# farhad-dalirani/StereoVision-SLAM

Hardware: AMD Instinct MI355X
Metric: stereo frames/sec (track + local BA), KITTI-00-shaped synthetic stereo 1241x376 (620x188 after the reference's 1/2 decimation) (higher is better)
Workload: dtype u8/i32 fixed-point (pyramid, LK), f32 (GFTT), f64 (LM, BA)

## Files before the change

### stereovision-slam_amd/csrc/k_lk.h

```cpp
#pragma once
#include "dev_common.h"

struct LkJob { int prev_slot, next_slot, pt_ofs, npts; };
struct LkParams {
    int max_level;
    int max_count;
    double eps2;
    double min_eig_thr;
    int use_initial_flow;
    float eig_num_thr;
    int eig_use_div;
    int njobs, blocks_per_job;
};

#define LK_WIN 11
#define LK_NPIX 121
#define LK_W_BITS 14
#define LK_REG 32
#ifndef LK_WAVES_PER_BLOCK
#define LK_WAVES_PER_BLOCK 1
#endif
#define LK_IROW 20

typedef uint32_t lk_u32_ua __attribute__((aligned(1)));
typedef uint16_t lk_u16_ua __attribute__((aligned(1)));
typedef short lk_s2 __attribute__((ext_vector_type(2)));

__device__ __forceinline__ int lk_dot2(uint32_t a, uint32_t b, int c)
{
    int r;
    asm("v_dot2_i32_i16 %0, %1, %2, %3" : "=v"(r) : "v"(a), "v"(b), "v"(c));
    return r;
}
#define LK_PAIR_SEL0 0x0c010c00u
__device__ __forceinline__ uint32_t lk_pair_sel(int a) { return LK_PAIR_SEL0 + (uint32_t)(a & 3) * 0x00010001u; }
__device__ __forceinline__ uint32_t lk_pair_at(const uint32_t *base32, int a, uint32_t sel)
{
    const uint32_t *q = base32 + (a >> 2);
    return __builtin_amdgcn_perm(q[1], q[0], sel);
}

__device__ __forceinline__ int lk_floor_i(float x)
{
    int r;
    asm("v_cvt_flr_i32_f32 %0, %1" : "=v"(r) : "v"(x));
    return r;
}

struct LkW { uint32_t top, bot; };

__device__ __forceinline__ LkW lk_weights(float a, float b)
{
    typedef float lk_f2 __attribute__((ext_vector_type(2)));
    const float S = (float)(1 << LK_W_BITS), M = 12582912.f;
    const float A = a * S, An = S - A, bn = 1.f - b;
    const lk_f2 p0 = (lk_f2){An, A} * (lk_f2){bn, bn} + (lk_f2){M, M};
    const uint32_t b00 = __float_as_uint(p0.x), b01 = __float_as_uint(p0.y), b10 = __float_as_uint(An * b + M);
    const uint32_t w11 = ((1u << LK_W_BITS) + 3u * 0x4B400000u) - (b00 + b01 + b10);
    LkW w;
    w.top = __builtin_amdgcn_perm(b01, b00, 0x05040100u);
    w.bot = __builtin_amdgcn_perm(w11, b10, 0x05040100u);
    return w;
}

__device__ __forceinline__ int lk_sample_u8(const uint32_t *base32, int a, int row_stride, LkW w)
{
    const uint32_t sel = lk_pair_sel(a);
    const uint32_t *q = base32 + (a >> 2);
    const int rs = row_stride >> 2;
    const uint32_t t = __builtin_amdgcn_perm(q[1], q[0], sel), b = __builtin_amdgcn_perm(q[rs + 1], q[rs], sel);
    return lk_dot2(t, w.top, lk_dot2(b, w.bot, 1 << (LK_W_BITS - 5 - 1))) >> (LK_W_BITS - 5);
}

__device__ __forceinline__ int lk_sample_diff(const uint32_t *base32, int a, int row_stride, LkW w, int acc0)
{
    const uint32_t sel = lk_pair_sel(a);
    const uint32_t *q = base32 + (a >> 2);
    const int rs = row_stride >> 2;
    const uint32_t t = __builtin_amdgcn_perm(q[1], q[0], sel), b = __builtin_amdgcn_perm(q[rs + 1], q[rs], sel);
    return lk_dot2(t, w.top, lk_dot2(b, w.bot, acc0)) >> (LK_W_BITS - 5);
}

typedef const __attribute__((address_space(3))) uint32_t *lk_lds_u32;
__device__ __forceinline__ int lk_sample_diff_at(uint32_t addr, LkW w, int acc0)
{
    lk_lds_u32 q = (lk_lds_u32)(uintptr_t)addr;
    const uint32_t t = q[0], b = q[LK_REG];
    return lk_dot2(t, w.top, lk_dot2(b, w.bot, acc0)) >> (LK_W_BITS - 5);
}

struct LkJRegs { uint32_t v[4]; };
__device__ __forceinline__ LkJRegs lk_stage_J_issue(const uint8_t *J0, uint32_t lofs, int pitch, int w, int h,
                                                    int cx, int cy, int lane, int &rx0, int &ry0)
{
    rx0 = __builtin_amdgcn_readfirstlane((cx - 10) & ~3);
    ry0 = __builtin_amdgcn_readfirstlane(cy - 10);
    const int r = lane >> 3, c4 = lane & 7;
    LkJRegs o;
    if (rx0 >= -SVS_BORDER && rx0 + LK_REG <= w + SVS_BORDER && ry0 >= -SVS_BORDER && ry0 + LK_REG <= h + SVS_BORDER) {
        const uint32_t p = lofs + (uint32_t)((ry0 + r) * pitch + (rx0 + c4 * 4));
#pragma unroll
        for (int k = 0; k < 4; ++k)
            o.v[k] = *reinterpret_cast<const uint32_t *>(J0 + (p + (uint32_t)(8 * k * pitch)));
    } else {
        const int gxmax = (w + SVS_BORDER - 4) & ~3;
        const int gx = max(-SVS_BORDER, min(rx0 + c4 * 4, gxmax));
#pragma unroll
        for (int k = 0; k < 4; ++k) {
            const int gy = max(-SVS_BORDER, min(ry0 + r + 8 * k, h + SVS_BORDER - 1));
            o.v[k] = *reinterpret_cast<const uint32_t *>(J0 + (lofs + (uint32_t)(gy * pitch + gx)));
        }
    }
    return o;
}
__device__ __forceinline__ void lk_stage_J_commit(uint32_t *sJ, const LkJRegs &o, int lane)
{
    typedef uint32_t lk_u4 __attribute__((ext_vector_type(4)));
    const int r = lane >> 3, c4 = lane & 7;
#pragma unroll
    for (int k = 0; k < 4; ++k) {
        const uint32_t cur = o.v[k];
        const uint32_t nxt = (uint32_t)__builtin_amdgcn_update_dpp(0, (int)cur, 0x101 , 0xf, 0xf, true);
        lk_u4 pr;
        pr.x = __builtin_amdgcn_perm(nxt, cur, 0x0c010c00u);
        pr.y = __builtin_amdgcn_perm(nxt, cur, 0x0c020c01u);
        pr.z = __builtin_amdgcn_perm(nxt, cur, 0x0c030c02u);
        pr.w = __builtin_amdgcn_perm(nxt, cur, 0x0c040c03u);
        *reinterpret_cast<lk_u4 *>(sJ + (r + 8 * k) * LK_REG + 4 * c4) = pr;
    }
    __builtin_amdgcn_fence(__ATOMIC_RELEASE, "wavefront");
    __builtin_amdgcn_wave_barrier();
}
__device__ __forceinline__ void lk_stage_J(uint32_t *sJ, const uint8_t *J0, uint32_t lofs, int pitch, int w, int h,
                                           int cx, int cy, int lane, int &rx0, int &ry0)
{
    const LkJRegs o = lk_stage_J_issue(J0, lofs, pitch, w, h, cx, cy, lane, rx0, ry0);
    lk_stage_J_commit(sJ, o, lane);
}

__device__ __forceinline__ float lk_sum_to_f32(long long s, float scale)
{
    const int lo = (int)s;
    const bool fits = (long long)lo == s;
    const int t = fits ? lo : (int)((s >> 1) | (s & 1));
    const uint32_t kb = fits ? __float_as_uint(scale) : __float_as_uint(2.f * scale);
    return (float)t * __uint_as_float(kb);
}

typedef unsigned lk_u2 __attribute__((ext_vector_type(2)));
__device__ __forceinline__ int lk_row_reduce(int w)
{
    w += dpp_i32<SVS_DPP_XOR1>(w);
    w += dpp_i32<SVS_DPP_XOR2>(w);
    w += dpp_i32<SVS_DPP_HALF_MIRROR>(w);
    w += dpp_i32<SVS_DPP_MIRROR>(w);
    return w;
}
__device__ __forceinline__ void lk_wave_sum2_i32(int a, int b, int &sa, int &sb)
{
    const lk_u2 r = __builtin_amdgcn_permlane16_swap((unsigned)a, (unsigned)b, false, false);
    const int v = (int)(r.x + r.y);
    const int w = lk_row_reduce(v);
    sa = __builtin_amdgcn_readlane(w, 0) + __builtin_amdgcn_readlane(w, 32);
    sb = __builtin_amdgcn_readlane(w, 16) + __builtin_amdgcn_readlane(w, 48);
}
__device__ __forceinline__ void lk_wave_sum4_i32(int a, int b, int c, int d, int &sa, int &sb, int &sc, int &sd)
{
    const lk_u2 r1 = __builtin_amdgcn_permlane16_swap((unsigned)a, (unsigned)b, false, false);
    const lk_u2 r2 = __builtin_amdgcn_permlane16_swap((unsigned)c, (unsigned)d, false, false);
    const int v1 = (int)(r1.x + r1.y), v2 = (int)(r2.x + r2.y);
    const lk_u2 q = __builtin_amdgcn_permlane32_swap((unsigned)v1, (unsigned)v2, false, false);
    const int w = lk_row_reduce((int)(q.x + q.y));
    sa = __builtin_amdgcn_readlane(w, 0);
    sb = __builtin_amdgcn_readlane(w, 16);
    sc = __builtin_amdgcn_readlane(w, 32);
    sd = __builtin_amdgcn_readlane(w, 48);
}

#ifndef LK_OCC_TEST
#define LK_OCC_TEST 0
#endif
#if LK_OCC_TEST == 1
#define LK_OCC_ATTR __attribute__((amdgpu_waves_per_eu(8, 8)))
#else
#define LK_OCC_ATTR
#endif
__global__ void __launch_bounds__(64 * LK_WAVES_PER_BLOCK) LK_OCC_ATTR
k_lk(const LkJob *jobs, const uint8_t *pyr, PyrGeom g, const float2 *prev_xy, float2 *next_xy,
     uint8_t *status, float *err, LkParams prm)
{
    __shared__ uint32_t sI_all[LK_WAVES_PER_BLOCK][16 * LK_IROW / 4 + 2];
    __shared__ uint32_t sD_all[LK_WAVES_PER_BLOCK][144];
    __shared__ __attribute__((aligned(16))) uint32_t sJ_all[LK_WAVES_PER_BLOCK][LK_REG * LK_REG];

#if LK_OCC_TEST == 2
    __shared__ uint32_t sPad[8192];
    sPad[threadIdx.x] = threadIdx.x;
    if (prm.max_count < 0) status[0] = (uint8_t)sPad[(threadIdx.x * 37) & 8191];
#endif
    const int wave = threadIdx.x >> 6, lane = threadIdx.x & 63;
    const int slot = blockIdx.x >> 3, round = slot / prm.blocks_per_job;
    const int job = round * 8 + (blockIdx.x & 7);
    if (job >= prm.njobs) return;
    const LkJob jb = jobs[job];
    const int pi = (slot - round * prm.blocks_per_job) * LK_WAVES_PER_BLOCK + wave;
    if (pi >= jb.npts) return;
    const int pt = jb.pt_ofs + pi;
    uint32_t *sI32 = sI_all[wave];
    uint32_t *sD = sD_all[wave];
    uint32_t *sJ = sJ_all[wave];

    const uint8_t *slotI = pyr + (size_t)jb.prev_slot * g.slot_bytes;
    const uint8_t *slotJ = pyr + (size_t)jb.next_slot * g.slot_bytes;

    const float2 prevp = prev_xy[pt];
    float2 nextp = next_xy[pt];
    bool st = true;
    float errv = 0.f;

    const int p0 = lane, p1 = lane + 64;
    const bool has1 = p1 < LK_NPIX;
    const int wy0 = p0 / LK_WIN, wx0 = p0 - wy0 * LK_WIN;
    const int wy1 = has1 ? p1 / LK_WIN : 0, wx1 = has1 ? p1 - wy1 * LK_WIN : 0;
    const int oI0 = (wy0 + 1) * LK_IROW + wx0 + 1, oI1 = (wy1 + 1) * LK_IROW + wx1 + 1;
    const int oD0 = wy0 * 12 + wx0, oD1 = wy1 * 12 + wx1;
    const int oJ0 = wy0 * LK_REG + wx0, oJ1 = wy1 * LK_REG + wx1;
    const uint32_t aJ0 = (uint32_t)(uintptr_t)(__attribute__((address_space(3))) uint32_t *)sJ + 4u * (uint32_t)oJ0,
                   aJ1 = (uint32_t)(uintptr_t)(__attribute__((address_space(3))) uint32_t *)sJ + 4u * (uint32_t)oJ1;
    const int sr = lane >> 2, sc = (lane & 3) * 3;
    const float FLT_SCALE = 1.f / (float)(1 << 20);
    const float e_lo = (float)(prm.eps2 * (1.0 - 2e-6)), e_hi = (float)(prm.eps2 * (1.0 + 2e-6));

    int max_level = prm.max_level;
    if (max_level > g.nlevels - 1) max_level = g.nlevels - 1;

    for (int level = max_level; level >= 0; --level) {
        const int w = g.w[level], h = g.h[level], pitch = g.pitch[level];
        const uint32_t lofs = (uint32_t)g.ofs[level] + (uint32_t)(SVS_BORDER * pitch + SVS_BORDER);
        const float lscale = __uint_as_float((uint32_t)(127 - level) << 23);
        float px = prevp.x * lscale, py = prevp.y * lscale;
        float nx, ny;
        if (level == max_level) {
            if (prm.use_initial_flow) { nx = nextp.x * lscale; ny = nextp.y * lscale; }
            else { nx = px; ny = py; }
        } else { nx = nextp.x * 2.f; ny = nextp.y * 2.f; }
        nextp.x = nx; nextp.y = ny;

        px -= 5.f; py -= 5.f;
        const int ipx = __builtin_amdgcn_readfirstlane(lk_floor_i(px)), ipy = __builtin_amdgcn_readfirstlane(lk_floor_i(py));
        const uint32_t wext = (uint32_t)(w + LK_WIN), hext = (uint32_t)(h + LK_WIN);
        if ((uint32_t)(ipx + LK_WIN) >= wext || (uint32_t)(ipy + LK_WIN) >= hext) {
            if (level == 0) { st = false; errv = 0.f; }
            continue;
        }
        const LkW iw = lk_weights(px - (float)ipx, py - (float)ipy);

        const int xs = (ipx - 1) & ~3, a0 = (ipx - 1) & 3;
        __builtin_amdgcn_wave_barrier();
        nx -= 5.f; ny -= 5.f;
        int rx0, ry0;
        LkJRegs jr;
        {
            const uint32_t ib = lofs + (uint32_t)((ipy - 1) * pitch + xs);
            const uint32_t v0 = *reinterpret_cast<const uint32_t *>(slotI + (ib + (uint32_t)((lane >> 2) * pitch + (lane & 3) * 4)));
            const uint32_t v1 = *reinterpret_cast<const uint32_t *>(slotI + (ib + (uint32_t)((lane & 15) * pitch + 16)));
            jr = lk_stage_J_issue(slotJ, lofs, pitch, w, h, lk_floor_i(nx), lk_floor_i(ny), lane, rx0, ry0);
            sI32[(lane >> 2) * (LK_IROW / 4) + (lane & 3)] = v0;
            sI32[(lane & 15) * (LK_IROW / 4) + 4] = v1;
        }
        __builtin_amdgcn_fence(__ATOMIC_RELEASE, "wavefront");
        __builtin_amdgcn_wave_barrier();
        if (lane < 48) {
            const int ab = sr * LK_IROW + a0 + sc;
            const int k8 = (ab & 3) * 8;
            const uint32_t *q = sI32 + (ab >> 2);
            const uint32_t al = q[0], ah = q[1], bl = q[LK_IROW / 4], bh = q[LK_IROW / 4 + 1],
                           cl = q[2 * (LK_IROW / 4)], ch = q[2 * (LK_IROW / 4) + 1];
            const uint32_t a4 = __builtin_amdgcn_alignbyte(ah, al, ab & 3), b4 = __builtin_amdgcn_alignbyte(bh, bl, ab & 3),
                           c4 = __builtin_amdgcn_alignbyte(ch, cl, ab & 3);
            auto pr = [](uint32_t v) -> lk_s2 { return __builtin_bit_cast(lk_s2, v); };
            const lk_s2 A01 = pr(__builtin_amdgcn_perm(0u, a4, 0x0c010c00u)), A23 = pr(__builtin_amdgcn_perm(0u, a4, 0x0c030c02u)), A4 = pr((ah >> k8) & 0xffu);
            const lk_s2 B01 = pr(__builtin_amdgcn_perm(0u, b4, 0x0c010c00u)), B23 = pr(__builtin_amdgcn_perm(0u, b4, 0x0c030c02u)), B4 = pr((bh >> k8) & 0xffu);
            const lk_s2 C01 = pr(__builtin_amdgcn_perm(0u, c4, 0x0c010c00u)), C23 = pr(__builtin_amdgcn_perm(0u, c4, 0x0c030c02u)), C4 = pr((ch >> k8) & 0xffu);
            const lk_s2 k3 = { 3, 3 }, k10 = { 10, 10 };
            const lk_s2 T001 = (A01 + C01) * k3 + B01 * k10, T023 = (A23 + C23) * k3 + B23 * k10, T04 = (A4 + C4) * k3 + B4 * k10;
            const lk_s2 T101 = C01 - A01, T123 = C23 - A23, T14 = C4 - A4;
            const lk_s2 DX01 = T023 - T001, DX2 = T04 - T023;
            const lk_s2 M01 = pr(__builtin_amdgcn_alignbyte(__builtin_bit_cast(uint32_t, T123), __builtin_bit_cast(uint32_t, T101), 2));
            const lk_s2 M2 = pr(__builtin_amdgcn_alignbyte(__builtin_bit_cast(uint32_t, T14), __builtin_bit_cast(uint32_t, T123), 2));
            const lk_s2 DY01 = (T123 + T101) * k3 + M01 * k10, DY2 = (T14 + T123) * k3 + M2 * k10;
            const uint32_t dx01 = __builtin_bit_cast(uint32_t, DX01), dy01 = __builtin_bit_cast(uint32_t, DY01);
            const uint32_t o0 = __builtin_amdgcn_perm(dy01, dx01, 0x05040100u), o1 = __builtin_amdgcn_perm(dy01, dx01, 0x07060302u),
                           o2 = __builtin_amdgcn_perm(__builtin_bit_cast(uint32_t, DY2), __builtin_bit_cast(uint32_t, DX2), 0x05040100u);
            const bool rowin = (uint32_t)(ipy + sr) < (uint32_t)h;
            sD[sr * 12 + sc + 0] = o0 & (0u - (uint32_t)(rowin & ((uint32_t)(ipx + sc + 0) < (uint32_t)w)));
            sD[sr * 12 + sc + 1] = o1 & (0u - (uint32_t)(rowin & ((uint32_t)(ipx + sc + 1) < (uint32_t)w)));
            sD[sr * 12 + sc + 2] = o2 & (0u - (uint32_t)(rowin & ((uint32_t)(ipx + sc + 2) < (uint32_t)w)));
        }
        __builtin_amdgcn_fence(__ATOMIC_RELEASE, "wavefront");
        __builtin_amdgcn_wave_barrier();
        int iv0, ix0, iy0, iv1, ix1, iy1;
        {
            iv0 = lk_sample_u8(sI32, oI0 + a0, LK_IROW, iw);
            const uint32_t d00 = sD[oD0], d01 = sD[oD0 + 1], d10 = sD[oD0 + 12], d11 = sD[oD0 + 13];
            ix0 = lk_dot2(__builtin_amdgcn_perm(d01, d00, 0x05040100u), iw.top,
                          lk_dot2(__builtin_amdgcn_perm(d11, d10, 0x05040100u), iw.bot, 1 << (LK_W_BITS - 1))) >> LK_W_BITS;
            iy0 = lk_dot2(__builtin_amdgcn_perm(d01, d00, 0x07060302u), iw.top,
                          lk_dot2(__builtin_amdgcn_perm(d11, d10, 0x07060302u), iw.bot, 1 << (LK_W_BITS - 1))) >> LK_W_BITS;
        }
        {
            iv1 = lk_sample_u8(sI32, oI1 + a0, LK_IROW, iw);
            const uint32_t d00 = sD[oD1], d01 = sD[oD1 + 1], d10 = sD[oD1 + 12], d11 = sD[oD1 + 13];
            ix1 = lk_dot2(__builtin_amdgcn_perm(d01, d00, 0x05040100u), iw.top,
                          lk_dot2(__builtin_amdgcn_perm(d11, d10, 0x05040100u), iw.bot, 1 << (LK_W_BITS - 1))) >> LK_W_BITS;
            iy1 = lk_dot2(__builtin_amdgcn_perm(d01, d00, 0x07060302u), iw.top,
                          lk_dot2(__builtin_amdgcn_perm(d11, d10, 0x07060302u), iw.bot, 1 << (LK_W_BITS - 1))) >> LK_W_BITS;
            if (!has1) { ix1 = 0; iy1 = 0; }
        }
        int sA11, sA12, sA22, sIdle;
        lk_wave_sum4_i32(__mul24(ix0, ix0) + __mul24(ix1, ix1), __mul24(ix0, iy0) + __mul24(ix1, iy1), __mul24(iy0, iy0) + __mul24(iy1, iy1), 0,
                         sA11, sA12, sA22, sIdle);
        const float A11 = (float)sA11 * FLT_SCALE, A12 = (float)sA12 * FLT_SCALE, A22 = (float)sA22 * FLT_SCALE;
        float D = A11 * A22 - A12 * A12;
        const float dd = A11 - A22;
        const float q2 = dd * dd + 4.f * A12 * A12;
        float eigNum;
        if (prm.eig_use_div) eigNum = A22 + A11 - sqrtf(q2);
        else {
            const float sq = __builtin_amdgcn_sqrtf(q2);
            eigNum = A22 + A11 - sq;
            if (fabsf(eigNum - prm.eig_num_thr) <= sq * 4.8e-7f + 1e-30f) eigNum = A22 + A11 - sqrtf(q2);
        }
        const bool eigSmall = prm.eig_use_div ? (double)(eigNum / (float)(2 * LK_WIN * LK_WIN)) < prm.min_eig_thr : eigNum < prm.eig_num_thr;
        if (eigSmall || D < 1.1920928955078125e-07f) {
            if (level == 0) st = false;
            continue;
        }
        D = 1.f / D;
        const bool narrow = sA11 <= 570000000 && sA22 <= 570000000;
        const int acc00 = (1 << (LK_W_BITS - 5 - 1)) - (iv0 << (LK_W_BITS - 5)), acc01 = (1 << (LK_W_BITS - 5 - 1)) - (iv1 << (LK_W_BITS - 5));
        const uint32_t ixx = __builtin_amdgcn_perm((uint32_t)ix1, (uint32_t)ix0, 0x05040100u), iyy = __builtin_amdgcn_perm((uint32_t)iy1, (uint32_t)iy0, 0x05040100u);
        float pdx = 0.f, pdy = 0.f, dx = 0.f, dy = 0.f;
        const float Ds = D * FLT_SCALE;
        bool moved = false, osc = false;
        lk_stage_J_commit(sJ, jr, lane);

        for (int j = 0; j < prm.max_count; ++j) {
            const int inx = __builtin_amdgcn_readfirstlane(lk_floor_i(nx)), iny = __builtin_amdgcn_readfirstlane(lk_floor_i(ny));
            if ((uint32_t)(inx + LK_WIN) >= wext || (uint32_t)(iny + LK_WIN) >= hext) {
                if (level == 0) st = false;
                break;
            }
            int ox = inx - rx0, oy = iny - ry0;
            if ((uint32_t)ox > LK_REG - 12 || (uint32_t)oy > LK_REG - 12) {
                lk_stage_J(sJ, slotJ, lofs, pitch, w, h, inx, iny, lane, rx0, ry0);
                ox = inx - rx0; oy = iny - ry0;
            }
            const LkW jw = lk_weights(nx - (float)inx, ny - (float)iny);
            const uint32_t jo = 4u * (uint32_t)(oy * LK_REG + ox);
            const int d0 = lk_sample_diff_at(aJ0 + jo, jw, acc00);
            const int d1 = lk_sample_diff_at(aJ1 + jo, jw, acc01);
            const uint32_t dd01 = __builtin_amdgcn_perm((uint32_t)d1, (uint32_t)d0, 0x05040100u);
            const int pb1 = lk_dot2(dd01, ixx, 0), pb2 = lk_dot2(dd01, iyy, 0);
            float b1, b2;
            if (narrow) {
                int s1, s2;
                lk_wave_sum2_i32(pb1, pb2, s1, s2);
                b1 = (float)s1; b2 = (float)s2;
            } else {
                b1 = lk_sum_to_f32(wave_sum_i32_wide(pb1), 1.f); b2 = lk_sum_to_f32(wave_sum_i32_wide(pb2), 1.f);
            }
            dx = (A12 * b2 - A22 * b1) * Ds;
            dy = (A12 * b1 - A11 * b2) * Ds;
            nx += dx; ny += dy;
            moved = true;
            const float dd2 = dx * dx + dy * dy;
            if (dd2 < e_lo) break;
            if (dd2 <= e_hi && (double)dx * (double)dx + (double)dy * (double)dy <= prm.eps2) break;
            if (j > 0 && fabsf(dx + pdx) <= 0.01f && fabsf(dy + pdy) <= 0.01f) {
                osc = true;
                break;
            }
            pdx = dx; pdy = dy;
        }
        if (moved) {
            nextp.x = nx + 5.f; nextp.y = ny + 5.f;
            if (osc) { nextp.x -= dx * 0.5f; nextp.y -= dy * 0.5f; }
        }

        if (st && level == 0) {
            const float fx = nextp.x - 5.f, fy = nextp.y - 5.f;
            const int inx = __builtin_amdgcn_readfirstlane(lk_floor_i(fx)), iny = __builtin_amdgcn_readfirstlane(lk_floor_i(fy));
            if (inx < -LK_WIN || inx >= w || iny < -LK_WIN || iny >= h) {
                st = false;
                continue;
            }
            int ox = inx - rx0, oy = iny - ry0;
            if (ox < 0 || ox > LK_REG - 12 || oy < 0 || oy > LK_REG - 12) {
                lk_stage_J(sJ, slotJ, lofs, pitch, w, h, inx, iny, lane, rx0, ry0);
                ox = inx - rx0; oy = iny - ry0;
            }
            const LkW jw = lk_weights(fx - (float)inx, fy - (float)iny);
            const uint32_t jo = 4u * (uint32_t)(oy * LK_REG + ox);
            const int d0 = lk_sample_diff_at(aJ0 + jo, jw, 1 << (LK_W_BITS - 5 - 1)) - iv0;
            const int d1 = lk_sample_diff_at(aJ1 + jo, jw, 1 << (LK_W_BITS - 5 - 1)) - iv1;
            const int e = (d0 < 0 ? -d0 : d0) + (has1 ? (d1 < 0 ? -d1 : d1) : 0);
            const int serr = wave_sum_i32(e);
            errv = (float)serr * 1.f / (float)(32 * LK_WIN * LK_WIN);
        }
    }
    if (lane == 0) {
        next_xy[pt] = nextp;
        status[pt] = st ? 1 : 0;
        if (err) err[pt] = errv;
    }
}
```

Measured before the change: 590,000.

## Interpolate patch first then apply Scharr for interior LK windows

For windows fully inside the image, the kernel now bilinearly interpolates a 13x16 patch of the prev image once, then computes the value and Scharr gradients from that interpolated patch with integer arithmetic. This replaces per-pixel gradient computation followed by separate bilinear sampling of value, dx and dy. Border windows keep the old path. The reordering relies on linearity, but rounding may differ slightly from the previous fixed-point result. An optional debug counter for the two paths is also added, off by default.

```diff
diff --git a/stereovision-slam_amd/csrc/k_lk.h b/stereovision-slam_amd/csrc/k_lk.h
--- a/stereovision-slam_amd/csrc/k_lk.h
+++ b/stereovision-slam_amd/csrc/k_lk.h
@@ -21,6 +21,18 @@
 #define LK_WAVES_PER_BLOCK 1
 #endif
 #define LK_IROW 20
+#define LK_UROWS 13
+#define LK_USTRIDE 16
+#ifndef LK_COUNT_PATHS
+#define LK_COUNT_PATHS 0
+#endif
+#if LK_COUNT_PATHS
+__device__ unsigned int lk_dev_visits[2];
+extern "C" int svslam_debug_lk_visits(unsigned int out[2])
+{
+    return (int)hipMemcpyFromSymbol(out, HIP_SYMBOL(lk_dev_visits), 2 * sizeof(unsigned int), 0, hipMemcpyDeviceToHost);
+}
+#endif
 
 typedef uint32_t lk_u32_ua __attribute__((aligned(1)));
 typedef uint16_t lk_u16_ua __attribute__((aligned(1)));
@@ -177,6 +189,17 @@
     sd = __builtin_amdgcn_readlane(w, 48);
 }
 
+__device__ __forceinline__ void lk_interp_first(const uint32_t *u, int &iv, int &ix, int &iy)
+{
+    const int u00 = (int)u[0], u02 = (int)u[2], u10 = (int)u[LK_USTRIDE], u12 = (int)u[LK_USTRIDE + 2],
+              u20 = (int)u[2 * LK_USTRIDE], u22 = (int)u[2 * LK_USTRIDE + 2],
+              u01 = (int)u[1], u21 = (int)u[2 * LK_USTRIDE + 1], u11 = (int)u[LK_USTRIDE + 1];
+    const int P = u22 - u00, Q = u02 - u20;
+    iv = u11 >> (LK_W_BITS - 5);
+    ix = (__mul24(P + Q, 3) + (__mul24(u12 - u10, 10) + (1 << (LK_W_BITS - 1)))) >> LK_W_BITS;
+    iy = (__mul24(P - Q, 3) + (__mul24(u21 - u01, 10) + (1 << (LK_W_BITS - 1)))) >> LK_W_BITS;
+}
+
 #ifndef LK_OCC_TEST
 #define LK_OCC_TEST 0
 #endif
@@ -190,7 +213,7 @@
      uint8_t *status, float *err, LkParams prm)
 {
     __shared__ uint32_t sI_all[LK_WAVES_PER_BLOCK][16 * LK_IROW / 4 + 2];
-    __shared__ uint32_t sD_all[LK_WAVES_PER_BLOCK][144];
+    __shared__ __attribute__((aligned(16))) uint32_t sD_all[LK_WAVES_PER_BLOCK][LK_UROWS * LK_USTRIDE];
     __shared__ __attribute__((aligned(16))) uint32_t sJ_all[LK_WAVES_PER_BLOCK][LK_REG * LK_REG];
 
 #if LK_OCC_TEST == 2
@@ -224,6 +247,7 @@
     const int wy1 = has1 ? p1 / LK_WIN : 0, wx1 = has1 ? p1 - wy1 * LK_WIN : 0;
     const int oI0 = (wy0 + 1) * LK_IROW + wx0 + 1, oI1 = (wy1 + 1) * LK_IROW + wx1 + 1;
     const int oD0 = wy0 * 12 + wx0, oD1 = wy1 * 12 + wx1;
+    const int oU0 = wy0 * LK_USTRIDE + wx0, oU1 = wy1 * LK_USTRIDE + wx1;
     const int oJ0 = wy0 * LK_REG + wx0, oJ1 = wy1 * LK_REG + wx1;
     const uint32_t aJ0 = (uint32_t)(uintptr_t)(__attribute__((address_space(3))) uint32_t *)sJ + 4u * (uint32_t)oJ0,
                    aJ1 = (uint32_t)(uintptr_t)(__attribute__((address_space(3))) uint32_t *)sJ + 4u * (uint32_t)oJ1;
@@ -270,52 +294,80 @@
         }
         __builtin_amdgcn_fence(__ATOMIC_RELEASE, "wavefront");
         __builtin_amdgcn_wave_barrier();
-        if (lane < 48) {
-            const int ab = sr * LK_IROW + a0 + sc;
-            const int k8 = (ab & 3) * 8;
-            const uint32_t *q = sI32 + (ab >> 2);
-            const uint32_t al = q[0], ah = q[1], bl = q[LK_IROW / 4], bh = q[LK_IROW / 4 + 1],
-                           cl = q[2 * (LK_IROW / 4)], ch = q[2 * (LK_IROW / 4) + 1];
-            const uint32_t a4 = __builtin_amdgcn_alignbyte(ah, al, ab & 3), b4 = __builtin_amdgcn_alignbyte(bh, bl, ab & 3),
-                           c4 = __builtin_amdgcn_alignbyte(ch, cl, ab & 3);
-            auto pr = [](uint32_t v) -> lk_s2 { return __builtin_bit_cast(lk_s2, v); };
-            const lk_s2 A01 = pr(__builtin_amdgcn_perm(0u, a4, 0x0c010c00u)), A23 = pr(__builtin_amdgcn_perm(0u, a4, 0x0c030c02u)), A4 = pr((ah >> k8) & 0xffu);
-            const lk_s2 B01 = pr(__builtin_amdgcn_perm(0u, b4, 0x0c010c00u)), B23 = pr(__builtin_amdgcn_perm(0u, b4, 0x0c030c02u)), B4 = pr((bh >> k8) & 0xffu);
-            const lk_s2 C01 = pr(__builtin_amdgcn_perm(0u, c4, 0x0c010c00u)), C23 = pr(__builtin_amdgcn_perm(0u, c4, 0x0c030c02u)), C4 = pr((ch >> k8) & 0xffu);
-            const lk_s2 k3 = { 3, 3 }, k10 = { 10, 10 };
-            const lk_s2 T001 = (A01 + C01) * k3 + B01 * k10, T023 = (A23 + C23) * k3 + B23 * k10, T04 = (A4 + C4) * k3 + B4 * k10;
-            const lk_s2 T101 = C01 - A01, T123 = C23 - A23, T14 = C4 - A4;
-            const lk_s2 DX01 = T023 - T001, DX2 = T04 - T023;
-            const lk_s2 M01 = pr(__builtin_amdgcn_alignbyte(__builtin_bit_cast(uint32_t, T123), __builtin_bit_cast(uint32_t, T101), 2));
-            const lk_s2 M2 = pr(__builtin_amdgcn_alignbyte(__builtin_bit_cast(uint32_t, T14), __builtin_bit_cast(uint32_t, T123), 2));
-            const lk_s2 DY01 = (T123 + T101) * k3 + M01 * k10, DY2 = (T14 + T123) * k3 + M2 * k10;
-            const uint32_t dx01 = __builtin_bit_cast(uint32_t, DX01), dy01 = __builtin_bit_cast(uint32_t, DY01);
-            const uint32_t o0 = __builtin_amdgcn_perm(dy01, dx01, 0x05040100u), o1 = __builtin_amdgcn_perm(dy01, dx01, 0x07060302u),
-                           o2 = __builtin_amdgcn_perm(__builtin_bit_cast(uint32_t, DY2), __builtin_bit_cast(uint32_t, DX2), 0x05040100u);
-            const bool rowin = (uint32_t)(ipy + sr) < (uint32_t)h;
-            sD[sr * 12 + sc + 0] = o0 & (0u - (uint32_t)(rowin & ((uint32_t)(ipx + sc + 0) < (uint32_t)w)));
-            sD[sr * 12 + sc + 1] = o1 & (0u - (uint32_t)(rowin & ((uint32_t)(ipx + sc + 1) < (uint32_t)w)));
-            sD[sr * 12 + sc + 2] = o2 & (0u - (uint32_t)(rowin & ((uint32_t)(ipx + sc + 2) < (uint32_t)w)));
-        }
-        __builtin_amdgcn_fence(__ATOMIC_RELEASE, "wavefront");
-        __builtin_amdgcn_wave_barrier();
         int iv0, ix0, iy0, iv1, ix1, iy1;
-        {
-            iv0 = lk_sample_u8(sI32, oI0 + a0, LK_IROW, iw);
-            const uint32_t d00 = sD[oD0], d01 = sD[oD0 + 1], d10 = sD[oD0 + 12], d11 = sD[oD0 + 13];
-            ix0 = lk_dot2(__builtin_amdgcn_perm(d01, d00, 0x05040100u), iw.top,
-                          lk_dot2(__builtin_amdgcn_perm(d11, d10, 0x05040100u), iw.bot, 1 << (LK_W_BITS - 1))) >> LK_W_BITS;
-            iy0 = lk_dot2(__builtin_amdgcn_perm(d01, d00, 0x07060302u), iw.top,
-                          lk_dot2(__builtin_amdgcn_perm(d11, d10, 0x07060302u), iw.bot, 1 << (LK_W_BITS - 1))) >> LK_W_BITS;
-        }
-        {
-            iv1 = lk_sample_u8(sI32, oI1 + a0, LK_IROW, iw);
-            const uint32_t d00 = sD[oD1], d01 = sD[oD1 + 1], d10 = sD[oD1 + 12], d11 = sD[oD1 + 13];
-            ix1 = lk_dot2(__builtin_amdgcn_perm(d01, d00, 0x05040100u), iw.top,
-                          lk_dot2(__builtin_amdgcn_perm(d11, d10, 0x05040100u), iw.bot, 1 << (LK_W_BITS - 1))) >> LK_W_BITS;
-            iy1 = lk_dot2(__builtin_amdgcn_perm(d01, d00, 0x07060302u), iw.top,
-                          lk_dot2(__builtin_amdgcn_perm(d11, d10, 0x07060302u), iw.bot, 1 << (LK_W_BITS - 1))) >> LK_W_BITS;
+        const bool interior = ipx >= 0 && ipx <= w - 12 && ipy >= 0 && ipy <= h - 12;
+#if LK_COUNT_PATHS
+        if (lane == 0) atomicAdd(&lk_dev_visits[interior ? 0 : 1], 1u);
+#endif
+        if (interior) {
+            if (lane < 4 * LK_UROWS) {
+                typedef uint32_t lk_u4 __attribute__((ext_vector_type(4)));
+                const uint32_t *q = sI32 + (lane >> 2) * (LK_IROW / 4) + (lane & 3);
+                const uint32_t tl = q[0], th = q[1], bl = q[LK_IROW / 4], bh = q[LK_IROW / 4 + 1];
+                const uint32_t s0 = LK_PAIR_SEL0 + (uint32_t)a0 * 0x00010001u;
+                const int rnd = 1 << (LK_W_BITS - 5 - 1);
+                lk_u4 u;
+                u.x = (uint32_t)lk_dot2(__builtin_amdgcn_perm(th, tl, s0), iw.top, lk_dot2(__builtin_amdgcn_perm(bh, bl, s0), iw.bot, rnd));
+                u.y = (uint32_t)lk_dot2(__builtin_amdgcn_perm(th, tl, s0 + 0x00010001u), iw.top,
+                                        lk_dot2(__builtin_amdgcn_perm(bh, bl, s0 + 0x00010001u), iw.bot, rnd));
+                u.z = (uint32_t)lk_dot2(__builtin_amdgcn_perm(th, tl, s0 + 0x00020002u), iw.top,
+                                        lk_dot2(__builtin_amdgcn_perm(bh, bl, s0 + 0x00020002u), iw.bot, rnd));
+                u.w = (uint32_t)lk_dot2(__builtin_amdgcn_perm(th, tl, s0 + 0x00030003u), iw.top,
+                                        lk_dot2(__builtin_amdgcn_perm(bh, bl, s0 + 0x00030003u), iw.bot, rnd));
+                *reinterpret_cast<lk_u4 *>(sD + (lane >> 2) * LK_USTRIDE + 4 * (lane & 3)) = u;
+            }
+            __builtin_amdgcn_fence(__ATOMIC_RELEASE, "wavefront");
+            __builtin_amdgcn_wave_barrier();
+            lk_interp_first(sD + oU0, iv0, ix0, iy0);
+            lk_interp_first(sD + oU1, iv1, ix1, iy1);
             if (!has1) { ix1 = 0; iy1 = 0; }
+        } else {
+            if (lane < 48) {
+                const int ab = sr * LK_IROW + a0 + sc;
+                const int k8 = (ab & 3) * 8;
+                const uint32_t *q = sI32 + (ab >> 2);
+                const uint32_t al = q[0], ah = q[1], bl = q[LK_IROW / 4], bh = q[LK_IROW / 4 + 1],
+                               cl = q[2 * (LK_IROW / 4)], ch = q[2 * (LK_IROW / 4) + 1];
+                const uint32_t a4 = __builtin_amdgcn_alignbyte(ah, al, ab & 3), b4 = __builtin_amdgcn_alignbyte(bh, bl, ab & 3),
+                               c4 = __builtin_amdgcn_alignbyte(ch, cl, ab & 3);
+                auto pr = [](uint32_t v) -> lk_s2 { return __builtin_bit_cast(lk_s2, v); };
+                const lk_s2 A01 = pr(__builtin_amdgcn_perm(0u, a4, 0x0c010c00u)), A23 = pr(__builtin_amdgcn_perm(0u, a4, 0x0c030c02u)), A4 = pr((ah >> k8) & 0xffu);
+                const lk_s2 B01 = pr(__builtin_amdgcn_perm(0u, b4, 0x0c010c00u)), B23 = pr(__builtin_amdgcn_perm(0u, b4, 0x0c030c02u)), B4 = pr((bh >> k8) & 0xffu);
+                const lk_s2 C01 = pr(__builtin_amdgcn_perm(0u, c4, 0x0c010c00u)), C23 = pr(__builtin_amdgcn_perm(0u, c4, 0x0c030c02u)), C4 = pr((ch >> k8) & 0xffu);
+                const lk_s2 k3 = { 3, 3 }, k10 = { 10, 10 };
+                const lk_s2 T001 = (A01 + C01) * k3 + B01 * k10, T023 = (A23 + C23) * k3 + B23 * k10, T04 = (A4 + C4) * k3 + B4 * k10;
+                const lk_s2 T101 = C01 - A01, T123 = C23 - A23, T14 = C4 - A4;
+                const lk_s2 DX01 = T023 - T001, DX2 = T04 - T023;
+                const lk_s2 M01 = pr(__builtin_amdgcn_alignbyte(__builtin_bit_cast(uint32_t, T123), __builtin_bit_cast(uint32_t, T101), 2));
+                const lk_s2 M2 = pr(__builtin_amdgcn_alignbyte(__builtin_bit_cast(uint32_t, T14), __builtin_bit_cast(uint32_t, T123), 2));
+                const lk_s2 DY01 = (T123 + T101) * k3 + M01 * k10, DY2 = (T14 + T123) * k3 + M2 * k10;
+                const uint32_t dx01 = __builtin_bit_cast(uint32_t, DX01), dy01 = __builtin_bit_cast(uint32_t, DY01);
+                const uint32_t o0 = __builtin_amdgcn_perm(dy01, dx01, 0x05040100u), o1 = __builtin_amdgcn_perm(dy01, dx01, 0x07060302u),
+                               o2 = __builtin_amdgcn_perm(__builtin_bit_cast(uint32_t, DY2), __builtin_bit_cast(uint32_t, DX2), 0x05040100u);
+                const bool rowin = (uint32_t)(ipy + sr) < (uint32_t)h;
+                sD[sr * 12 + sc + 0] = o0 & (0u - (uint32_t)(rowin & ((uint32_t)(ipx + sc + 0) < (uint32_t)w)));
+                sD[sr * 12 + sc + 1] = o1 & (0u - (uint32_t)(rowin & ((uint32_t)(ipx + sc + 1) < (uint32_t)w)));
+                sD[sr * 12 + sc + 2] = o2 & (0u - (uint32_t)(rowin & ((uint32_t)(ipx + sc + 2) < (uint32_t)w)));
+            }
+            __builtin_amdgcn_fence(__ATOMIC_RELEASE, "wavefront");
+            __builtin_amdgcn_wave_barrier();
+            {
+                iv0 = lk_sample_u8(sI32, oI0 + a0, LK_IROW, iw);
+                const uint32_t d00 = sD[oD0], d01 = sD[oD0 + 1], d10 = sD[oD0 + 12], d11 = sD[oD0 + 13];
+                ix0 = lk_dot2(__builtin_amdgcn_perm(d01, d00, 0x05040100u), iw.top,
+                              lk_dot2(__builtin_amdgcn_perm(d11, d10, 0x05040100u), iw.bot, 1 << (LK_W_BITS - 1))) >> LK_W_BITS;
+                iy0 = lk_dot2(__builtin_amdgcn_perm(d01, d00, 0x07060302u), iw.top,
+                              lk_dot2(__builtin_amdgcn_perm(d11, d10, 0x07060302u), iw.bot, 1 << (LK_W_BITS - 1))) >> LK_W_BITS;
+            }
+            {
+                iv1 = lk_sample_u8(sI32, oI1 + a0, LK_IROW, iw);
+                const uint32_t d00 = sD[oD1], d01 = sD[oD1 + 1], d10 = sD[oD1 + 12], d11 = sD[oD1 + 13];
+                ix1 = lk_dot2(__builtin_amdgcn_perm(d01, d00, 0x05040100u), iw.top,
+                              lk_dot2(__builtin_amdgcn_perm(d11, d10, 0x05040100u), iw.bot, 1 << (LK_W_BITS - 1))) >> LK_W_BITS;
+                iy1 = lk_dot2(__builtin_amdgcn_perm(d01, d00, 0x07060302u), iw.top,
+                              lk_dot2(__builtin_amdgcn_perm(d11, d10, 0x07060302u), iw.bot, 1 << (LK_W_BITS - 1))) >> LK_W_BITS;
+                if (!has1) { ix1 = 0; iy1 = 0; }
+            }
         }
         int sA11, sA12, sA22, sIdle;
         lk_wave_sum4_i32(__mul24(ix0, ix0) + __mul24(ix1, ix1), __mul24(ix0, iy0) + __mul24(ix1, iy1), __mul24(iy0, iy0) + __mul24(iy1, iy1), 0,
```

Result: no change. 600,500 (median of 6 runs) (+1.8%).
